# eddyxzc/lpopc

Hardware: AMD Instinct MI355X
Metric: eval_g+eval_jac_g calls/sec, 4-phase 4096-LGR-pt problem (higher is better)
Workload: dtype f64

## Files before the change

### lpopc_amd/csrc/rpm_ipm.hpp

```cpp
#pragma once
#include <string>
#include <vector>

#include "rpm_engine.hpp"

namespace rpm {

struct KktSubHost {
  int Nt, Nb, nb, b, CS;
  long long koff;
  int roff;
};

struct IpmPlan {
  int n = 0, m = 0, ns = 0, nv = 0;
  int Nt = 0, Nb = 0, nb = 0;
  int b = 0, CS = 0;
  std::vector<int> pos;
  std::vector<int> row_slack;
  std::vector<int> slack_row;
  std::vector<int> fixed;
  std::vector<int> jac_dst, hes_dst;
  std::vector<int> diag_dst;
  std::vector<int> slk_dst;
// ... 23 lines not shown
  }
};

int build_ipm_plan(Engine& e, IpmPlan& p, std::string* why, int nested = 0);
void ipm_plan_group_hessian(IpmPlan& p);
long long ipm_plan_offset(const IpmPlan& p, int ua, int uc);

#if defined(__HIP__) || defined(__HIPCC__)
#define RPM_IPM_HD __host__ __device__
#else
#define RPM_IPM_HD
#endif

constexpr int IPM_W = 16;
constexpr int IPM_LONG_COLUMN = 256;
constexpr int IPM_FILL_CHUNK = 4096;
constexpr int IPM_DENSE_SLOTS = 22, IPM_DENSE_TILE_WAVES = 7, IPM_DENSE_LDS_ROW = 18;
constexpr int IPM_DENSE_TILES = IPM_DENSE_SLOTS * IPM_DENSE_TILE_WAVES;
constexpr int IPM_DENSE_ROWS = 17, IPM_DENSE_EARLY = 4;
static_assert(IPM_DENSE_ROWS * (IPM_DENSE_ROWS + 1) / 2 <= IPM_DENSE_TILES, "resident tiles");
RPM_IPM_HD inline int ipm_dense_early(int block_rows) { return block_rows > IPM_DENSE_ROWS ? block_rows - IPM_DENSE_ROWS : 0; }
RPM_IPM_HD inline int ipm_dense_tile(int block_rows, int I, int Kb) {
  const int E = ipm_dense_early(block_rows), R = block_rows - E;
  if (Kb >= E) { const int kr = Kb - E; return kr * R - kr * (kr - 1) / 2 + I - Kb; }
  return R * (R + 1) / 2 + Kb * block_rows - Kb * (Kb - 1) / 2 + I - Kb;
}
RPM_IPM_HD inline int ipm_dense_tiles_of(int block_rows) { return block_rows * (block_rows + 1) / 2; }

inline size_t ipm_factor_lds_bytes(int b, int nb) {
  const size_t W = IPM_W;
// ... 21 lines not shown
struct IpmFillList {
  std::vector<int> dst, ki, hg, ptr;
  bool one_pass = false;
  int n_chunks() const { return one_pass ? int(ptr.size()) - 1 : 0; }
};
IpmFillList ipm_fill_list(const IpmPlan& p);

struct IpmFusedFill {
  bool built = false;
  int tiles = IPM_DENSE_TILES;
  std::vector<int> ptr, ki, hg, live;
  std::vector<unsigned long long> map;
};
IpmFusedFill ipm_fused_fill(const IpmSubList& s, const IpmFillList& fill);

}
```

### lpopc_amd/csrc/rpm_ipm_device.hpp

```cpp
#pragma once
#include <hip/hip_runtime.h>

#include "rpm_ipm.hpp"

namespace rpm {

constexpr int IPM_FMAX = 1024;
constexpr int IPM_TRACE = 8;
constexpr double IPM_INF = 1e19;
constexpr int IPM_LB_H = 6;
constexpr int IPM_LB_PART = 80 * 16;
constexpr int IPM_LB_SMALL = 8 + 2 * (2 * IPM_LB_H) * (2 * IPM_LB_H) + 2 * (2 * IPM_LB_H);

struct IpmOpts {
  double tol = 1e-8, mu_init = 0.1, kappa_eps = 10.0, kappa_mu = 0.2, theta_mu = 1.5, tau_min = 0.99;
  double bound_push = 1e-2, bound_frac = 1e-2, kappa_sigma = 1e10, s_max = 100.0;
  double ws_bound_push = 1e-3, ws_bound_frac = 1e-3, ws_slack_bound_push = 1e-3, ws_slack_bound_frac = 1e-3;
  double ws_mult_bound_push = 1e-3, ws_mult_init_max = 1e6;
  double gamma_theta = 1e-5, gamma_phi = 1e-8, eta_phi = 1e-8, delta = 1.0, s_theta = 1.1, s_phi = 2.3, gamma_alpha = 0.05;
  double delta_c = 1e-9, delta_w_first = 1e-4, delta_w_min = 1e-20, delta_w_max = 1e40, kw_inc_first = 100.0, kw_inc = 8.0,
         kw_dec = 1.0 / 3.0;
  int max_iter = 3000, max_ls = 40;
  double acceptable_tol = 1e-6;
  int acceptable_iter = 15;
// ... 20 lines not shown
  int status;
  int iter, nfilt, accepted, refactor, npos, nneg, nbad, ls, armijo, nzb, pad;
  int mode, resto_it, enter_resto, n_resto;
  int n_acc, skip_update;
  double th0, zeta;
  double mu_r, th_r, thr_max, thr_min, phi_r;
  int nrfilt, soc_on, soc_req, soc_p, use_soc, n_soc;
  double alpha_soc, az_soc, th_old_soc;
  double mu_max, refs[4];
  int fixed_mode, nrefs;
  int n_recalc, ic_hot;
  double th_trial, phi_trial;
  long long dbg[8];
};

struct IpmDev {
  int B, n, m, ns, nv, Nt, Nb, nb, b, CS, nnz_jac, nnz_h;
  long long sg, sv, kstride;
  const int *pos, *row_slack, *slack_row, *jac_dst, *hes_dst, *diag_dst, *slk_dst, *jt_ptr, *jt_ent, *jt_row;
  const int *hg_ptr, *hg_src, *hg_dst;
  int n_hg;
  const int *as_dst, *as_ki, *as_hg, *as_ptr;
  int as_nchunk;
  const int* long_cols;
  int n_long;
  const double *gl, *gu;
  double *v, *vl, *vu, *zL, *zU, *lam, *dv, *dlam, *dzL, *dzU, *glag, *c, *rhs, *K, *filt;
  double *xe, *xt, *grad, *g, *jac, *hess, *obj, *gt, *objt;
  double *vR, *dr2;
  double *vl0, *vu0;
// ... 7 lines not shown
  IpmInst* inst;
  int* cnt;
  IpmOpts o;
  const KktSub* subs;
  int n_sub, n_l1, n_l2;
  int* piv;
  const int *cg_ptr, *cg_src, *cg_dst;
  const int *rg_ptr, *rg_src, *rg_dst;
  const int *rs_dst, *rs_src;
  const int* gap_pos;
  int n_cg, n_rg, n_rs, n_gap;
  const int *cg2_ptr, *cg2_src, *cg2_dst, *rg2_ptr, *rg2_src, *rg2_dst, *rs2_dst, *rs2_src;
  int n_cg2, n_rg2, n_rs2;
  int n_cg_long, n_cg2_long;
  int max_sub_nt;
  int df_tiles;
  size_t l1_dense_lds;
  int last_dense_corner;
  size_t l2_dense_lds, last_dense_lds;
  int df_on;
  const int *df_ptr, *df_ki, *df_hg, *as_live;
  int as_nlive;
  const unsigned long long* df_map;
  int rhs_mult;
  int lb_on;
  double *lb_S, *lb_Y;
  double *lb_xprev;
  double *lb_gold;
  int scal_on;
  double *sc, *sf, *lam_h;
// ... 28 lines not shown
void ipm_launch_scale_lambda(const IpmDev& D, hipStream_t st);
void ipm_launch_scale_hessian(const IpmDev& D, hipStream_t st);
void ipm_launch_unscale_lambda(const IpmDev& D, double* out, hipStream_t st);
void lb_launch_reset(const IpmDev& D, hipStream_t st);
void lb_launch_update(const IpmDev& D, hipStream_t st);
void lb_launch_columns_and_solve(const IpmDev& D, hipStream_t st);
void lb_launch_small(const IpmDev& D, hipStream_t st);
void lb_launch_correct(const IpmDev& D, int check_status, hipStream_t st);
void ipm_launch_jt_lambda_into(const IpmDev& D, double* out, hipStream_t st);
size_t kkt_factor_lds_bytes(const IpmPlan& p);
hipError_t kkt_factor_prepare(int tiles_per_wave, size_t lds_bytes);
size_t kkt_factor_dense_lds_bytes(int block_rows);
int kkt_factor_dense_max_block_rows();
hipError_t kkt_factor_dense_prepare(size_t lds_bytes);
void kkt_launch_factor(const IpmDev& D, int tiles_per_wave, size_t lds_bytes, hipStream_t st);
void kkt_launch_solve(const IpmDev& D, int check_status, hipStream_t st, int forward_done = 0);
int kkt_level1_fused(const IpmDev& D);
void kkt_launch_vec(const IpmDev& D, unsigned n_rhs, const int* dst, const int* src, int n, int mode, int check_status, hipStream_t st);

}
```

### lpopc_amd/csrc/rpm_ipm_solver.hip

```cpp
#include <algorithm>
#include <cstdlib>
#include <cstring>
#include <memory>
#include <new>

#include "rpm_ipm_solver.hpp"

using namespace rpm;

namespace {
struct IpmAllocs {
  rpm_ipm* h;
  int rc = RPM_OK;
  template <class T>
  void room(T** dst, size_t count) { if (!rc) rc = ipm_alloc(h, dst, count); }
  template <class T>
  void table(const T** dst, const std::vector<T>& src) {
    T* p = nullptr;
    if (!rc) rc = ipm_alloc(h, &p, src.size(), src.data());
    *dst = p;
  }
};

bool env_is_zero(const char* name) {
// ... 36 lines not shown
    a.table(&D.as_live, fused.live); a.table(&D.df_map, fused.map);
    D.as_nlive = int(fused.live.size());
  }
  a.table(&D.subs, s.subs);
  D.n_sub = int(s.subs.size()); D.n_l1 = s.n_l1; D.n_l2 = s.n_l2; D.max_sub_nt = s.max_sub_nt;
  a.room(&D.piv, size_t(D.B) * s.subs.size() * 3);
  a.table(&D.cg_ptr, p.cg_ptr); a.table(&D.cg_src, p.cg_src); a.table(&D.cg_dst, p.cg_dst);
  a.table(&D.rg_ptr, p.rg_ptr); a.table(&D.rg_src, p.rg_src); a.table(&D.rg_dst, p.rg_dst);
  a.table(&D.rs_dst, p.rs_dst); a.table(&D.rs_src, p.rs_src); a.table(&D.gap_pos, p.gap_pos);
  D.n_cg = int(p.cg_dst.size()); D.n_rg = int(p.rg_dst.size()); D.n_rs = int(p.rs_dst.size()); D.n_gap = int(p.gap_pos.size());
  a.table(&D.cg2_ptr, p.cg2_ptr); a.table(&D.cg2_src, p.cg2_src); a.table(&D.cg2_dst, p.cg2_dst);
  a.table(&D.rg2_ptr, p.rg2_ptr); a.table(&D.rg2_src, p.rg2_src); a.table(&D.rg2_dst, p.rg2_dst);
  a.table(&D.rs2_dst, p.rs2_dst); a.table(&D.rs2_src, p.rs2_src);
  D.n_cg2 = int(p.cg2_dst.size()); D.n_rg2 = int(p.rg2_dst.size()); D.n_rs2 = int(p.rs2_dst.size());
  D.n_cg_long = p.n_cg_long; D.n_cg2_long = p.n_cg2_long;
  return a.rc;
}

int alloc_state(rpm_ipm* h) {
  Engine& e = h->eng->e;
  const IpmPlan& p = h->plan;
  IpmDev& D = h->D;
  const size_t B = size_t(D.B), Bm = B * size_t(std::max(p.m, 1));
  IpmAllocs a{h};
  a.room(&D.v, B * p.nv); a.room(&D.vl, B * p.nv); a.room(&D.vu, B * p.nv);
  a.room(&D.zL, B * p.nv); a.room(&D.zU, B * p.nv); a.room(&D.lam, B * p.m);
  a.room(&D.dv, B * p.nv); a.room(&D.dlam, B * p.m); a.room(&D.dzL, B * p.nv);
  a.room(&D.dzU, B * p.nv); a.room(&D.glag, B * p.nv); a.room(&D.c, B * p.m);
  a.room(&D.rhs, B * size_t(p.Nt_alloc)); a.room(&D.K, B * size_t(p.storage())); a.room(&D.filt, B * 2 * IPM_FMAX);
  a.room(&D.xe, B * p.n); a.room(&D.xt, B * p.n); a.room(&D.grad, B * p.n);
// ... 162 lines not shown
  }
  else if (k == "restoration_penalty") o.resto_rho = value;
  else if (k == "level1_dense") {
    if (value != 0.0 && !h->l1_dense_lds) { h->err = "level1_dense: no nested dissection, or an interval block of more than 21 block rows"; return RPM_E_UNSUPPORTED; }
    h->D.l1_dense_lds = value != 0.0 ? h->l1_dense_lds : 0;
  }
  else if (k == "upper_dense") {
    h->D.l2_dense_lds = value != 0.0 ? h->l2_dense_lds : 0;
    h->D.last_dense_lds = value != 0.0 ? h->last_dense_lds : 0;
    h->D.last_dense_corner = value == 2.0 ? 0 : 1;
  }
  else if (k == "fused_fill") {
    if (value != 0.0 && !h->D.df_map) { h->err = "fused_fill: level 1 does not run on kkt_factor_dense_kernel"; return RPM_E_UNSUPPORTED; }
    h->D.df_on = value != 0.0;
  }
  else if (k == "trace") {
    const int cap = int(value);
    if (cap < 0 || cap > 100000) { h->err = "trace: 0 ... 100000 records"; return RPM_E_INVALID; }
    h->D.trace = nullptr;
    h->D.trace_cap = 0;
    if (cap > 0) {
      int rc = ipm_alloc(h, &h->D.trace, size_t(h->D.B) * cap * IPM_TRACE);
      if (rc) return rc;
      h->D.trace_cap = cap;
    }
  }
  else { h->err = "unknown option " + k; return RPM_E_INVALID; }
  return RPM_OK;
}

// ... 325 lines not shown
```

### lpopc_amd/csrc/rpm_ipm_solver.hpp

```cpp
#pragma once
#include <algorithm>
#include <cstdio>
#include <string>
#include <vector>

#include "rpm_device_internal.hpp"
#include "rpm_ipm_device.hpp"

struct rpm_ipm {
  rpm_engine* eng = nullptr;
  rpm::IpmPlan plan;
  rpm::IpmDev D{};
  std::vector<void*> allocs;
  int* h_cnt = nullptr;
  size_t factor_lds = 0;
  size_t l1_dense_lds = 0;
  size_t l2_dense_lds = 0, last_dense_lds = 0;
  int factor_mt = rpm::IPM_MT;
  std::string err;
  std::vector<rpm::IpmInst> h_inst;
  int total_factorizations = 0, total_iterations = 0, total_trials = 0, total_soc = 0;
  hipEvent_t ev[4] = {nullptr, nullptr, nullptr, nullptr};
  double factor_ms = 0.0, solve_ms = 0.0;
  bool solve_pending = false;
  bool attached = false;
  bool lbfgs = false;
  int lb_iterations = 0;
  bool solved = false;
  bool debug_started = false;
  int debug_ls = 0;
  double* d_host_form = nullptr;
  ~rpm_ipm() {
    if (attached && eng && eng->e.ipm_attached > 0) eng->e.ipm_attached -= 1;
// ... 21 lines not shown
  IPM_TRY(h, hipMalloc(&p, (count ? count : 1) * sizeof(T)));
  h->allocs.push_back(p);
  *dst = static_cast<T*>(p);
  if (src && count) IPM_TRY(h, hipMemcpy(p, src, count * sizeof(T), hipMemcpyHostToDevice));
  return RPM_OK;
}

inline int launch_check(rpm_ipm* h, const char* what) {
  hipError_t s = hipGetLastError();
  if (s != hipSuccess) {
    h->err = std::string(what) + ": " + hipGetErrorString(s);
    return RPM_E_DEVICE;
  }
  return RPM_OK;
}
inline int factor_and_solve_launch(rpm_ipm* h, hipStream_t st, bool factor, bool solve, int check_status, int forward_done = 0) {
  if (factor) kkt_launch_factor(h->D, h->factor_mt, h->factor_lds, st);
  if (solve) kkt_launch_solve(h->D, check_status, st, forward_done);
  return launch_check(h, "kkt kernels");
}

int ipm_check_start_args(rpm_ipm* h, const char* who, const char* need, bool warm, const void* x, const void* lambda, const void* z_L,
                         const void* z_U);
int ipm_start(rpm_ipm* h, bool warm, const double* d_x, const double* d_lambda, const double* d_zL, const double* d_zU, hipStream_t st);
int host_form(rpm_ipm* h, double** d_x, double** d_l, double** d_zL, double** d_zU);

inline int ipm_abi_status(int device_status) {
  return device_status == 1 ? 0 : (device_status == 6 ? 1 : device_status);
}

struct IpmLoop {
  rpm_ipm* h;
  Engine& e;
// ... 35 lines not shown
      ipm_launch_inertia(D, st);
      h->total_factorizations += 1;
      if ((rc = fetch_counts())) return rc;
      float ms = 0.f;
      if (hipEventElapsedTime(&ms, h->ev[0], h->ev[1]) == hipSuccess) h->factor_ms += ms;
      if (h->h_cnt[1] == 0) break;
    }
    return RPM_OK;
  }
  int substitute() const {
    IPM_TRY(h, hipEventRecord(h->ev[2], st));
    if (h->lbfgs && h->lb_iterations > 0) {
      lb_launch_columns_and_solve(D, st);
      lb_launch_small(D, st);
    }
    if (int rc = factor_and_solve_launch(h, st, false, true, 1, 1)) return rc;
    if (h->lbfgs) lb_launch_correct(D, 1, st);
    IPM_TRY(h, hipEventRecord(h->ev[3], st));
    h->solve_pending = true;
    return RPM_OK;
  }
  int direction() const {
    IPM_TRY(h, hipMemsetAsync(D.cnt + 2, 0, 2 * sizeof(int), st));
    ipm_launch_direction(D, st);
    h->h_cnt[3] = 0;
    return RPM_OK;
  }
  int line_search_round(double* soc_rhs_copy = nullptr) const {
    int rc;
    if (h->h_cnt[3] > 0) {
      ipm_launch_soc_rhs(D, st);
      if (soc_rhs_copy)
        IPM_TRY(h, hipMemcpyAsync(soc_rhs_copy, D.rhs, size_t(D.B) * size_t(h->plan.Nt_alloc) * sizeof(double), hipMemcpyDeviceToHost, st));
      if ((rc = factor_and_solve_launch(h, st, false, true, 2))) return rc;
      if (h->lbfgs) lb_launch_correct(D, 2, st);
      ipm_launch_soc_direction(D, st);
      h->total_soc += 1;
    }
// ... 67 lines not shown
```

### lpopc_amd/csrc/rpm_ipm_tables.cpp

```cpp
#include <algorithm>
#include <unordered_map>

#include "rpm_ipm.hpp"

namespace rpm {

IpmSubList ipm_sub_list(const IpmPlan& p) {
  IpmSubList s;
  if (p.nd) {
    for (const KktSubHost& g : p.subs) s.subs.push_back(KktSub{KktGeom{g.Nt, g.Nb, g.nb, g.b, g.CS}, g.roff, g.koff});
    s.n_l2 = p.n_l2;
    s.n_l1 = int(s.subs.size()) - 1 - s.n_l2;
  } else {
    s.subs.push_back(KktSub{KktGeom{p.Nt, p.Nb, p.nb, p.b, p.CS}, 0, 0});
  }
  for (const KktSub& q : s.subs) s.max_sub_nt = std::max(s.max_sub_nt, q.g.Nt);
  return s;
}

std::vector<int> ipm_long_columns(const IpmPlan& p) {
  std::vector<int> cols;
  for (int i = 0; i < p.n; ++i)
    if (p.jt_ptr[size_t(i) + 1] - p.jt_ptr[size_t(i)] > IPM_LONG_COLUMN) cols.push_back(i);
  return cols;
// ... 77 lines not shown
        t.ki.push_back(fill.ki[q]);
        t.hg.push_back(fill.hg[q]);
      }
    }
    e2 = e3;
    if (size_t(number) + 1 > 2 * size_t(NTB) * IPM_W * IPM_DENSE_LDS_ROW) return none;
    for (long long c = (k0 + IPM_FILL_CHUNK - 1) / IPM_FILL_CHUNK; (c + 1) * IPM_FILL_CHUNK <= k1; ++c) skip[size_t(c)] = 1;
  }
  t.ptr[3 * size_t(s.n_l1)] = int(t.ki.size());
  for (int c = 0; c < fill.n_chunks(); ++c)
    if (!skip[size_t(c)]) t.live.push_back(c);
  t.built = true;
  return t;
}

}
```

### lpopc_amd/csrc/rpm_kkt_solve.hip

```cpp
#include <algorithm>
#include <cmath>
#include <cstring>
#include <new>

#include "rpm_device_internal.hpp"
#include "rpm_ipm_device.hpp"

namespace rpm {

__device__ inline void block_range(const KktGeom& G, int J0, int* J1, int* nrb, int* nr) {
  if (J0 < G.Nb) {
    *J1 = min(J0 + IPM_W, G.Nb);
    const int last = min(*J1 - 1 + G.b, G.Nb - 1);
    *nrb = max(last - *J1 + 1, 0);
    *nr = *nrb + G.nb;
  } else {
    *J1 = min(J0 + IPM_W, G.Nt);
    *nrb = 0;
    *nr = G.Nt - *J1;
  }
}
__device__ inline int panel_row(const KktGeom& G, int J0, int J1, int nrb, int q) {
  return J0 >= G.Nb ? J1 + q : (q < nrb ? J1 + q : G.Nb + (q - nrb));
}

template <bool RL, int PF = 1>
__global__ __launch_bounds__(256) void kkt_solve_kernel(const double* Kall, long long kstride, const KktSub* subs, int sub0, int n_here,
                                                        const IpmInst* inst, double* rhs_all, long long rhs_stride, int check_status,
                                                        int phase, int kmod) {
  constexpr int W = IPM_W;
#define SOLVE_BARRIER() do { if (RL) asm volatile("s_waitcnt lgkmcnt(0)\n\ts_barrier" ::: "memory"); else __syncthreads(); } while (0)
  const int bi = blockIdx.x / n_here, bk = bi % kmod, t = threadIdx.x, nt = blockDim.x;
  if (check_status && (inst[bk].status != 0 || (check_status == 2 && !inst[bk].soc_req))) return;
  const KktSub sub = subs[sub0 + int(blockIdx.x) % n_here];
  const KktGeom G = sub.g;
  const double* K = Kall + size_t(bk) * kstride + sub.koff;
  double* rg = rhs_all + size_t(bi) * rhs_stride + sub.roff;
  extern __shared__ double rsh[];
  double* r = RL ? rsh : rg;
  __shared__ double Dg[W * (W + 1)], ys[W], zs[W], red[4][W];
  const int di = t / W, dj = t % W;
  const int nbb = (G.Nb + W - 1) / W, ncb = (G.nb + W - 1) / W, nblk = nbb + ncb;
  if (RL) {
    for (int i = t; i < G.Nt; i += nt) rsh[i] = rg[i];
    SOLVE_BARRIER();
  }
  struct Blk { int J0, J1, nrb, nr, w; };
  auto blk_of = [&](int blk) {
    Blk B;
    B.J0 = blk < nbb ? blk * W : G.Nb + (blk - nbb) * W;
    block_range(G, B.J0, &B.J1, &B.nrb, &B.nr);
    B.w = B.J1 - B.J0;
    return B;
  };
  auto fetch = [&](int blk, double& dg, double (&l)[W]) {
    if (blk < 0 || blk >= nblk) return;
    const Blk B = blk_of(blk);
    dg = (di < B.w && dj <= di) ? K[G.at(B.J0 + di, B.J0 + dj)] : 0.0;
    const int row = t < B.nr ? panel_row(G, B.J0, B.J1, B.nrb, t) : -1;
    const bool brd = row >= G.Nb;
    const int kstep = brd ? G.CS : G.CS - 1;
    const double* kp = K + (size_t(B.J0) * G.CS + (brd ? G.b + 1 + row - G.Nb : max(row - B.J0, 0)));
#pragma unroll
    for (int c = 0; c < W; ++c)
      l[c] = (row >= 0 && c < B.w && (brd || row - (B.J0 + c) <= G.b)) ? kp[c * kstep] : 0.0;
  };
  double dg0, l0[W], dg1, l1[W];
  const int fwd_end = phase == 1 ? nbb : (phase == 2 ? 0 : nblk), bwd_begin = phase == 2 ? nbb : (phase == 1 ? 0 : nblk);
  auto forward_step = [&](int blk, double& dg, double (&l)[W]) {
    const Blk B = blk_of(blk);
    if (di < W && dj <= di) Dg[di * (W + 1) + dj] = dg;
    if (t < W) zs[t] = t < B.w ? r[B.J0 + t] : 0.0;
    SOLVE_BARRIER();
    if (t < W) {
      double y = zs[t];
#pragma unroll
      for (int k = 0; k < W; ++k)
        if (k < t && t < B.w) y = __builtin_fma(Dg[t * (W + 1) + k], zs[k], y);
      ys[t] = y;
      if (t < B.w) r[B.J0 + t] = y;
    }
    SOLVE_BARRIER();
    for (int q = t; q < B.nr; q += nt) {
      const int row = panel_row(G, B.J0, B.J1, B.nrb, q);
      double acc = 0.0;
#pragma unroll
      for (int c = 0; c < W; ++c) {
        const double lv = q == t ? l[c] : ((c < B.w && (row >= G.Nb || row - (B.J0 + c) <= G.b)) ? K[G.at(row, B.J0 + c)] : 0.0);
        acc = __builtin_fma(lv, ys[c], acc);
      }
      r[row] -= acc;
    }
    fetch(blk + PF, dg, l);
    SOLVE_BARRIER();
  };
  if (fwd_end > 0) { fetch(0, dg0, l0); if (PF == 2) fetch(1 < fwd_end ? 1 : -1, dg1, l1); }
  for (int blk = 0; blk < fwd_end; blk += PF) {
    forward_step(blk, dg0, l0);
    if (PF == 2 && blk + 1 < fwd_end) forward_step(blk + 1, dg1, l1);
  }
  auto backward_step = [&](int blk, double& dg, double (&l)[W]) {
    const Blk B = blk_of(blk);
    if (di < W && dj <= di) Dg[di * (W + 1) + dj] = dg;
    double p[W];
#pragma unroll
    for (int c = 0; c < W; ++c) p[c] = 0.0;
    for (int q = t; q < B.nr; q += nt) {
      const int row = panel_row(G, B.J0, B.J1, B.nrb, q);
      const double xr = r[row];
#pragma unroll
      for (int c = 0; c < W; ++c) {
        const double lv = q == t ? l[c] : ((c < B.w && (row >= G.Nb || row - (B.J0 + c) <= G.b)) ? K[G.at(row, B.J0 + c)] : 0.0);
        p[c] = __builtin_fma(lv, xr, p[c]);
      }
    }
    fetch(blk - PF, dg, l);
    {
      const int ln = t & 63;
      double q8[8], q4[4], q2[2], u;
      const bool h32 = ln & 32, h16 = ln & 16, h8 = ln & 8, h4 = ln & 4;
#pragma unroll
      for (int i = 0; i < 8; ++i) q8[i] = (h32 ? p[i + 8] : p[i]) + __shfl_xor(h32 ? p[i] : p[i + 8], 32);
#pragma unroll
      for (int i = 0; i < 4; ++i) q4[i] = (h16 ? q8[i + 4] : q8[i]) + __shfl_xor(h16 ? q8[i] : q8[i + 4], 16);
#pragma unroll
      for (int i = 0; i < 2; ++i) q2[i] = (h8 ? q4[i + 2] : q4[i]) + __shfl_xor(h8 ? q4[i] : q4[i + 2], 8);
      u = (h4 ? q2[1] : q2[0]) + __shfl_xor(h4 ? q2[0] : q2[1], 4);
      u += __shfl_xor(u, 2);
      u += __shfl_xor(u, 1);
      if ((ln & 3) == 0) red[t >> 6][ln >> 2] = u;
    }
    SOLVE_BARRIER();
    if (t < W) zs[t] = t < B.w ? r[B.J0 + t] / Dg[t * (W + 1) + t] - (red[0][t] + red[1][t] + red[2][t] + red[3][t]) : 0.0;
    SOLVE_BARRIER();
    if (t < B.w) {
      double x = zs[t];
#pragma unroll
      for (int k = 0; k < W; ++k)
        if (k > t && k < B.w) x = __builtin_fma(Dg[k * (W + 1) + t], zs[k], x);
      r[B.J0 + t] = x;
    }
    SOLVE_BARRIER();
  };
  if (bwd_begin > 0) { fetch(bwd_begin - 1, dg0, l0); if (PF == 2) fetch(bwd_begin - 2, dg1, l1); }
  for (int blk = bwd_begin - 1; blk >= 0; blk -= PF) {
    backward_step(blk, dg0, l0);
    if (PF == 2 && blk - 1 >= 0) backward_step(blk - 1, dg1, l1);
  }
  if (RL)
    for (int i = t; i < G.Nt; i += nt) rg[i] = rsh[i];
#undef SOLVE_BARRIER
}

__global__ __launch_bounds__(256) void ipm_inertia_kernel(IpmDev D) {
  const int bi = (blockIdx.x * blockDim.x + threadIdx.x) >> 6, lane = threadIdx.x & 63;
  if (bi >= D.B) return;
  IpmInst& S = D.inst[bi];
  if (S.status != 0 || !S.refactor) return;
  const IpmOpts& o = D.o;
// ... 36 lines not shown
}
__global__ void kkt_vec_kernel(double* vall, long long vstride, const int* __restrict__ dst, const int* __restrict__ src, int n, int mode,
                               const IpmInst* inst, int check_status, int kmod) {
  const int bi = blockIdx.y, bk = bi % kmod;
  if (check_status && (inst[bk].status != 0 || (check_status == 2 && !inst[bk].soc_req) || (check_status == 3 && !inst[bk].refactor))) return;
  double* v = vall + size_t(bi) * vstride;
  for (int i = blockIdx.x * blockDim.x + threadIdx.x; i < n; i += gridDim.x * blockDim.x) v[dst[i]] = mode ? v[src[i]] : 0.0;
}
void kkt_launch_vec(const IpmDev& D, unsigned n_rhs, const int* dst, const int* src, int n, int mode, int check_status, hipStream_t st) {
  if (!n) return;
  const unsigned blocks = unsigned(std::max(1, std::min(256, (n + 255) / 256)));
  hipLaunchKernelGGL(kkt_vec_kernel, dim3(blocks, n_rhs), dim3(256), 0, st, D.rhs, (long long)D.Nt, dst, src, n, mode, D.inst,
                     check_status, D.B);
}

static void launch_solve_subs(const IpmDev& D, int sub0, int n_here, int phase, int check_status, hipStream_t st) {
  const dim3 grid(unsigned(D.B) * unsigned(D.rhs_mult > 1 ? D.rhs_mult : 1) * unsigned(n_here));
  if (size_t(D.max_sub_nt) * sizeof(double) <= 48 * 1024 && grid.x <= 512)
    hipLaunchKernelGGL((kkt_solve_kernel<true, 2>), grid, dim3(256), size_t(D.max_sub_nt) * sizeof(double), st, D.K, D.kstride, D.subs, sub0, n_here,
                       D.inst, D.rhs, (long long)D.Nt, check_status, phase, D.B);
  else if (size_t(D.max_sub_nt) * sizeof(double) <= 48 * 1024)
    hipLaunchKernelGGL(kkt_solve_kernel<true>, grid, dim3(256), size_t(D.max_sub_nt) * sizeof(double), st, D.K, D.kstride, D.subs, sub0, n_here,
                       D.inst, D.rhs, (long long)D.Nt, check_status, phase, D.B);
  else
    hipLaunchKernelGGL(kkt_solve_kernel<false>, grid, dim3(256), 0, st, D.K, D.kstride, D.subs, sub0, n_here, D.inst, D.rhs, (long long)D.Nt,
                       check_status, phase, D.B);
}
void kkt_launch_solve(const IpmDev& D, int check_status, hipStream_t st, int forward_done) {
  const unsigned VB = unsigned(D.B) * unsigned(D.rhs_mult > 1 ? D.rhs_mult : 1);
  if (D.n_l1 == 0) {
    launch_solve_subs(D, 0, 1, 0, check_status, st);
    return;
  }
  auto vec = [&](const int* dst, const int* src, int n, int mode) { kkt_launch_vec(D, VB, dst, src, n, mode, check_status, st); };
  auto gather = [&](const int* ptr, const int* src, const int* dst, int n) {
    if (!n) return;
    const unsigned blocks = unsigned(std::max(1, std::min(4096, (n + 3) / 4)));
    hipLaunchKernelGGL(kkt_gather_seq_kernel, dim3(blocks, VB), dim3(256), 0, st, D.rhs, (long long)D.Nt, ptr, src, dst, n, D.inst, check_status, D.B);
  };
  if (!(forward_done && kkt_level1_fused(D))) {
    vec(D.gap_pos, nullptr, D.n_gap, 0);
    launch_solve_subs(D, 0, D.n_l1, 1, check_status, st);
  }
  gather(D.rg_ptr, D.rg_src, D.rg_dst, D.n_rg);
  if (D.n_l2) {
    launch_solve_subs(D, D.n_l1, D.n_l2, 1, check_status, st);
    gather(D.rg2_ptr, D.rg2_src, D.rg2_dst, D.n_rg2);
  }
  launch_solve_subs(D, D.n_l1 + D.n_l2, 1, 0, check_status, st);
  if (D.n_l2) {
    vec(D.rs2_dst, D.rs2_src, D.n_rs2, 1);
    launch_solve_subs(D, D.n_l1, D.n_l2, 2, check_status, st);
  }
  vec(D.rs_dst, D.rs_src, D.n_rs, 1);
  launch_solve_subs(D, 0, D.n_l1, 2, check_status, st);
}
void ipm_launch_inertia(const IpmDev& D, hipStream_t st) {
  hipLaunchKernelGGL(ipm_inertia_kernel, dim3(unsigned((D.B + 3) / 4)), dim3(256), 0, st, D);
}

}
```

Before: 653,900.

## Fuse inter-level KKT gather/copy glue and step staging into solve kernels

After: 651,600. No clear change (-0.3%).

```diff
diff --git a/lpopc_amd/csrc/rpm_ipm.hpp b/lpopc_amd/csrc/rpm_ipm.hpp
--- a/lpopc_amd/csrc/rpm_ipm.hpp
+++ b/lpopc_amd/csrc/rpm_ipm.hpp
@@ -61,6 +61,7 @@
 
 constexpr int IPM_W = 16;
 constexpr int IPM_LONG_COLUMN = 256;
+constexpr int IPM_GLUE_LONG = 16;
 constexpr int IPM_FILL_CHUNK = 4096;
 constexpr int IPM_DENSE_SLOTS = 22, IPM_DENSE_TILE_WAVES = 7, IPM_DENSE_LDS_ROW = 18;
 constexpr int IPM_DENSE_TILES = IPM_DENSE_SLOTS * IPM_DENSE_TILE_WAVES;
@@ -112,4 +113,11 @@
 };
 IpmFusedFill ipm_fused_fill(const IpmSubList& s, const IpmFillList& fill);
 
+struct IpmGlueTables {
+  bool built = false;
+  std::vector<int> g_sub, g_ptr, g_src, g_dst, c_sub, c_dst, c_src;
+  std::vector<int> l_ptr[2], l_src[2], l_dst[2];
+};
+IpmGlueTables ipm_glue_tables(const IpmPlan& p, const IpmSubList& s);
+
 }
diff --git a/lpopc_amd/csrc/rpm_ipm_device.hpp b/lpopc_amd/csrc/rpm_ipm_device.hpp
--- a/lpopc_amd/csrc/rpm_ipm_device.hpp
+++ b/lpopc_amd/csrc/rpm_ipm_device.hpp
@@ -58,6 +58,11 @@
   long long dbg[8];
 };
 
+struct KktGlue {
+  const int *g_sub, *g_ptr, *g_src, *g_dst, *c_sub, *c_dst, *c_src;
+  int on;
+};
+
 struct IpmDev {
   int B, n, m, ns, nv, Nt, Nb, nb, b, CS, nnz_jac, nnz_h;
   long long sg, sv, kstride;
@@ -95,6 +100,11 @@
   int n_cg2, n_rg2, n_rs2;
   int n_cg_long, n_cg2_long;
   int max_sub_nt;
+  KktGlue glue;
+  const int *gl_ptr[2], *gl_src[2], *gl_dst[2];
+  int n_gl[2];
+  int fused_steps;
+  int fused_sub;
   int df_tiles;
   size_t l1_dense_lds;
   int last_dense_corner;
@@ -153,7 +163,7 @@
 int kkt_factor_dense_max_block_rows();
 hipError_t kkt_factor_dense_prepare(size_t lds_bytes);
 void kkt_launch_factor(const IpmDev& D, int tiles_per_wave, size_t lds_bytes, hipStream_t st);
-void kkt_launch_solve(const IpmDev& D, int check_status, hipStream_t st, int forward_done = 0);
+void kkt_launch_solve(const IpmDev& D, int check_status, hipStream_t st, int forward_done = 0, int* zero_cnt = nullptr, int n_zero_cnt = 0);
 int kkt_level1_fused(const IpmDev& D);
 void kkt_launch_vec(const IpmDev& D, unsigned n_rhs, const int* dst, const int* src, int n, int mode, int check_status, hipStream_t st);
 
diff --git a/lpopc_amd/csrc/rpm_ipm_solver.hip b/lpopc_amd/csrc/rpm_ipm_solver.hip
--- a/lpopc_amd/csrc/rpm_ipm_solver.hip
+++ b/lpopc_amd/csrc/rpm_ipm_solver.hip
@@ -74,6 +74,19 @@
   a.table(&D.rs2_dst, p.rs2_dst); a.table(&D.rs2_src, p.rs2_src);
   D.n_cg2 = int(p.cg2_dst.size()); D.n_rg2 = int(p.rg2_dst.size()); D.n_rs2 = int(p.rs2_dst.size());
   D.n_cg_long = p.n_cg_long; D.n_cg2_long = p.n_cg2_long;
+  const IpmGlueTables glue = ipm_glue_tables(p, s);
+  h->glue_built = glue.built;
+  if (glue.built) {
+    a.table(&D.glue.g_sub, glue.g_sub); a.table(&D.glue.g_ptr, glue.g_ptr); a.table(&D.glue.g_src, glue.g_src); a.table(&D.glue.g_dst, glue.g_dst);
+    a.table(&D.glue.c_sub, glue.c_sub); a.table(&D.glue.c_dst, glue.c_dst); a.table(&D.glue.c_src, glue.c_src);
+    for (int st = 0; st < 2; ++st) {
+      a.table(&D.gl_ptr[st], glue.l_ptr[st]); a.table(&D.gl_src[st], glue.l_src[st]); a.table(&D.gl_dst[st], glue.l_dst[st]);
+      D.n_gl[st] = int(glue.l_dst[st].size());
+    }
+  }
+  D.fused_sub = 1;
+  D.fused_steps = 1;
+  D.glue.on = glue.built ? 1 : 0;
   return a.rc;
 }
 
@@ -266,6 +279,11 @@
     if (value != 0.0 && !h->D.df_map) { h->err = "fused_fill: level 1 does not run on kkt_factor_dense_kernel"; return RPM_E_UNSUPPORTED; }
     h->D.df_on = value != 0.0;
   }
+  else if (k == "fused_substitution") {
+    h->D.fused_sub = value == 1.0 || value == 3.0;
+    h->D.fused_steps = value == 1.0 || value == 2.0;
+    h->D.glue.on = h->D.fused_sub && h->glue_built;
+  }
   else if (k == "trace") {
     const int cap = int(value);
     if (cap < 0 || cap > 100000) { h->err = "trace: 0 ... 100000 records"; return RPM_E_INVALID; }
diff --git a/lpopc_amd/csrc/rpm_ipm_solver.hpp b/lpopc_amd/csrc/rpm_ipm_solver.hpp
--- a/lpopc_amd/csrc/rpm_ipm_solver.hpp
+++ b/lpopc_amd/csrc/rpm_ipm_solver.hpp
@@ -17,6 +17,7 @@
   size_t l1_dense_lds = 0;
   size_t l2_dense_lds = 0, last_dense_lds = 0;
   int factor_mt = rpm::IPM_MT;
+  bool glue_built = false;
   std::string err;
   std::vector<rpm::IpmInst> h_inst;
   int total_factorizations = 0, total_iterations = 0, total_trials = 0, total_soc = 0;
@@ -68,9 +69,10 @@
   }
   return RPM_OK;
 }
-inline int factor_and_solve_launch(rpm_ipm* h, hipStream_t st, bool factor, bool solve, int check_status, int forward_done = 0) {
+inline int factor_and_solve_launch(rpm_ipm* h, hipStream_t st, bool factor, bool solve, int check_status, int forward_done = 0,
+                                   int* zero_cnt = nullptr, int n_zero_cnt = 0) {
   if (factor) kkt_launch_factor(h->D, h->factor_mt, h->factor_lds, st);
-  if (solve) kkt_launch_solve(h->D, check_status, st, forward_done);
+  if (solve) kkt_launch_solve(h->D, check_status, st, forward_done, zero_cnt, n_zero_cnt);
   return launch_check(h, "kkt kernels");
 }
 
@@ -136,14 +138,14 @@
       lb_launch_columns_and_solve(D, st);
       lb_launch_small(D, st);
     }
-    if (int rc = factor_and_solve_launch(h, st, false, true, 1, 1)) return rc;
+    if (int rc = factor_and_solve_launch(h, st, false, true, 1, 1, D.fused_sub ? D.cnt + 2 : nullptr, 2)) return rc;
     if (h->lbfgs) lb_launch_correct(D, 1, st);
     IPM_TRY(h, hipEventRecord(h->ev[3], st));
     h->solve_pending = true;
     return RPM_OK;
   }
   int direction() const {
-    IPM_TRY(h, hipMemsetAsync(D.cnt + 2, 0, 2 * sizeof(int), st));
+    if (!D.fused_sub) IPM_TRY(h, hipMemsetAsync(D.cnt + 2, 0, 2 * sizeof(int), st));
     ipm_launch_direction(D, st);
     h->h_cnt[3] = 0;
     return RPM_OK;
diff --git a/lpopc_amd/csrc/rpm_ipm_tables.cpp b/lpopc_amd/csrc/rpm_ipm_tables.cpp
--- a/lpopc_amd/csrc/rpm_ipm_tables.cpp
+++ b/lpopc_amd/csrc/rpm_ipm_tables.cpp
@@ -115,4 +115,105 @@
   return t;
 }
 
-}
+IpmGlueTables ipm_glue_tables(const IpmPlan& p, const IpmSubList& s) {
+  IpmGlueTables none, t;
+  const int n_sub = int(s.subs.size());
+  if (s.n_l1 <= 0 || n_sub != s.n_l1 + s.n_l2 + 1) return none;
+  auto level_of = [&](int si) { return si < s.n_l1 ? 1 : (si < s.n_l1 + s.n_l2 ? 2 : 3); };
+  auto sub_of = [&](int row) {
+    int lo = 0, hi = n_sub;
+    while (hi - lo > 1) {
+      const int mid = (lo + hi) / 2;
+      if (s.subs[size_t(mid)].roff <= row) lo = mid; else hi = mid;
+    }
+    const KktSub& q = s.subs[size_t(lo)];
+    return row >= q.roff && row < q.roff + q.g.Nt ? lo : -1;
+  };
+  for (int si = 1; si < n_sub; ++si)
+    if (s.subs[size_t(si)].roff < s.subs[size_t(si) - 1].roff + s.subs[size_t(si) - 1].g.Nt) return none;
+  auto in_work_space = [&](int row, int si) { return si >= 0 && level_of(si) < 3 && row >= s.subs[size_t(si)].roff + s.subs[size_t(si)].g.Nb; };
+
+  {
+    size_t rows = 0;
+    for (int si = 0; si < s.n_l1 + s.n_l2; ++si) rows += size_t(s.subs[size_t(si)].g.nb);
+    if (p.gap_pos.size() != rows) return none;
+    std::vector<int> g = p.gap_pos;
+    std::sort(g.begin(), g.end());
+    for (size_t i = 0; i < g.size(); ++i)
+      if ((i > 0 && g[i] == g[i - 1]) || !in_work_space(g[i], sub_of(g[i]))) return none;
+  }
+
+  struct Dest { int sub, row; bool in_stage[2]; std::vector<int> src[2]; };
+  std::vector<Dest> dests;
+  std::unordered_map<int, size_t> dest_of_row;
+  auto add_stage = [&](const std::vector<int>& ptr, const std::vector<int>& src, const std::vector<int>& dst, int src_level) {
+    if (ptr.size() != dst.size() + 1 && !(dst.empty() && ptr.empty())) return false;
+    std::unordered_map<int, int> seen;
+    for (size_t i = 0; i < dst.size(); ++i) {
+      const int si = sub_of(dst[i]);
+      if (si < 0 || level_of(si) <= src_level || in_work_space(dst[i], si) || !seen.emplace(dst[i], 1).second) return false;
+      if (ptr[i] < 0 || ptr[i] > ptr[i + 1] || size_t(ptr[i + 1]) > src.size()) return false;
+      auto it = dest_of_row.find(dst[i]);
+      if (it == dest_of_row.end()) {
+        it = dest_of_row.emplace(dst[i], dests.size()).first;
+        dests.push_back(Dest{si, dst[i], {false, false}, {{}, {}}});
+      }
+      dests[it->second].in_stage[src_level - 1] = true;
+      for (int j = ptr[i]; j < ptr[i + 1]; ++j) {
+        const int ss = sub_of(src[size_t(j)]);
+        if (ss < 0 || level_of(ss) != src_level || !in_work_space(src[size_t(j)], ss)) return false;
+        dests[it->second].src[src_level - 1].push_back(src[size_t(j)]);
+      }
+    }
+    return true;
+  };
+  if (!add_stage(p.rg_ptr, p.rg_src, p.rg_dst, 1)) return none;
+  if (!add_stage(p.rg2_ptr, p.rg2_src, p.rg2_dst, 2)) return none;
+  std::stable_sort(dests.begin(), dests.end(), [](const Dest& a, const Dest& b) { return a.sub < b.sub; });
+  t.g_sub.assign(size_t(n_sub) + 1, 0);
+  t.g_ptr.push_back(0);
+  for (int st = 0; st < 2; ++st) t.l_ptr[st].push_back(0);
+  for (const Dest& d : dests) {
+    if (d.src[0].size() > size_t(IPM_GLUE_LONG) || d.src[1].size() > size_t(IPM_GLUE_LONG)) {
+      for (int st = 0; st < 2; ++st) {
+        if (!d.in_stage[st]) continue;
+        t.l_dst[st].push_back(d.row);
+        t.l_src[st].insert(t.l_src[st].end(), d.src[st].begin(), d.src[st].end());
+        t.l_ptr[st].push_back(int(t.l_src[st].size()));
+      }
+      continue;
+    }
+    t.g_sub[size_t(d.sub) + 1] += 1;
+    t.g_dst.push_back(d.row);
+    for (int st = 0; st < 2; ++st) t.g_src.insert(t.g_src.end(), d.src[st].begin(), d.src[st].end());
+    t.g_ptr.push_back(int(t.g_src.size()));
+  }
+  for (int si = 0; si < n_sub; ++si) t.g_sub[size_t(si) + 1] += t.g_sub[size_t(si)];
+
+  struct Copy { int sub, dst, src; };
+  std::vector<Copy> copies;
+  std::unordered_map<int, int> copied;
+  auto add_copies = [&](const std::vector<int>& dst, const std::vector<int>& src, int dst_level) {
+    if (dst.size() != src.size()) return false;
+    for (size_t i = 0; i < dst.size(); ++i) {
+      const int sd = sub_of(dst[i]), ss = sub_of(src[i]);
+      if (sd < 0 || level_of(sd) != dst_level || !in_work_space(dst[i], sd) || !copied.emplace(dst[i], 1).second) return false;
+      if (ss < 0 || level_of(ss) <= dst_level || in_work_space(src[i], ss)) return false;
+      copies.push_back(Copy{sd, dst[i], src[i]});
+    }
+    return true;
+  };
+  if (!add_copies(p.rs_dst, p.rs_src, 1) || !add_copies(p.rs2_dst, p.rs2_src, 2)) return none;
+  std::stable_sort(copies.begin(), copies.end(), [](const Copy& a, const Copy& b) { return a.sub < b.sub; });
+  t.c_sub.assign(size_t(n_sub) + 1, 0);
+  for (const Copy& c : copies) {
+    t.c_sub[size_t(c.sub) + 1] += 1;
+    t.c_dst.push_back(c.dst);
+    t.c_src.push_back(c.src);
+  }
+  for (int si = 0; si < n_sub; ++si) t.c_sub[size_t(si) + 1] += t.c_sub[size_t(si)];
+  t.built = true;
+  return t;
+}
+
+}
diff --git a/lpopc_amd/csrc/rpm_kkt_solve.hip b/lpopc_amd/csrc/rpm_kkt_solve.hip
--- a/lpopc_amd/csrc/rpm_kkt_solve.hip
+++ b/lpopc_amd/csrc/rpm_kkt_solve.hip
@@ -24,26 +24,83 @@
   return J0 >= G.Nb ? J1 + q : (q < nrb ? J1 + q : G.Nb + (q - nrb));
 }
 
-template <bool RL, int PF = 1>
+__device__ inline double lane_value(double v, int k) {
+  return __hiloint2double(__builtin_amdgcn_readlane(__double2hiint(v), k), __builtin_amdgcn_readlane(__double2loint(v), k));
+}
+
+template <bool RL, int PF = 1, bool FS = false>
 __global__ __launch_bounds__(256) void kkt_solve_kernel(const double* Kall, long long kstride, const KktSub* subs, int sub0, int n_here,
                                                         const IpmInst* inst, double* rhs_all, long long rhs_stride, int check_status,
-                                                        int phase, int kmod) {
+                                                        int phase, int kmod, KktGlue glue, int* zero_cnt, int n_zero_cnt) {
   constexpr int W = IPM_W;
 #define SOLVE_BARRIER() do { if (RL) asm volatile("s_waitcnt lgkmcnt(0)\n\ts_barrier" ::: "memory"); else __syncthreads(); } while (0)
   const int bi = blockIdx.x / n_here, bk = bi % kmod, t = threadIdx.x, nt = blockDim.x;
-  if (check_status && (inst[bk].status != 0 || (check_status == 2 && !inst[bk].soc_req))) return;
-  const KktSub sub = subs[sub0 + int(blockIdx.x) % n_here];
+  if (zero_cnt && blockIdx.x == 0 && t < n_zero_cnt) zero_cnt[t] = 0;
+  const int si = sub0 + int(blockIdx.x) % n_here;
+  const KktSub sub = subs[si];
+  const bool gathers = glue.on && phase != 2, copies = glue.on && phase == 2;
+  const int* list_of = gathers ? glue.g_sub : glue.c_sub;
+  const int list0 = glue.on ? list_of[si] : 0, list1 = glue.on ? list_of[si + 1] : 0;
+  const int inst_status = check_status ? inst[bk].status : 0, inst_soc = check_status == 2 ? inst[bk].soc_req : 1;
+  if (inst_status != 0 || !inst_soc) return;
   const KktGeom G = sub.g;
   const double* K = Kall + size_t(bk) * kstride + sub.koff;
   double* rg = rhs_all + size_t(bi) * rhs_stride + sub.roff;
   extern __shared__ double rsh[];
   double* r = RL ? rsh : rg;
-  __shared__ double Dg[W * (W + 1)], ys[W], zs[W], red[4][W];
+  __shared__ double Dg2[(FS ? 2 : 1) * W * (W + 1)], ys[W], zs[W], red[4][W];
   const int di = t / W, dj = t % W;
   const int nbb = (G.Nb + W - 1) / W, ncb = (G.nb + W - 1) / W, nblk = nbb + ncb;
+  constexpr int GB = 8;
+  const double* v = rhs_all + size_t(bi) * rhs_stride;
+  auto gather_fetch = [&](int j, int j1, double (&s)[GB]) {
+    int idx[GB];
+#pragma unroll
+    for (int u = 0; u < GB; ++u) idx[u] = j + u < j1 ? glue.g_src[j + u] : -1;
+#pragma unroll
+    for (int u = 0; u < GB; ++u) s[u] = idx[u] >= 0 ? v[idx[u]] : 0.0;
+  };
+  auto gather_add = [&](int j, int j1, const double (&s)[GB], double acc) {
+#pragma unroll
+    for (int u = 0; u < GB; ++u)
+      if (j + u < j1) acc += s[u];
+    return acc;
+  };
+  const bool zero_border = glue.on && phase == 1;
+  const int e0 = list0 + t, e1 = list1;
+  int gj0 = 0, gj1 = 0, gd = 0;
+  double gs[GB], cv = 0.0;
+  if (gathers && e0 < e1) {
+    gj0 = glue.g_ptr[e0]; gj1 = glue.g_ptr[e0 + 1]; gd = glue.g_dst[e0] - sub.roff;
+    gather_fetch(gj0, gj1, gs);
+  }
+  if (copies && e0 < e1) { gd = glue.c_dst[e0] - sub.roff; cv = v[glue.c_src[e0]]; }
   if (RL) {
-    for (int i = t; i < G.Nt; i += nt) rsh[i] = rg[i];
-    SOLVE_BARRIER();
+    for (int i = t; i < G.Nt; i += nt) rsh[i] = (zero_border && i >= G.Nb) ? 0.0 : rg[i];
+    SOLVE_BARRIER();
+  } else if (zero_border) {
+    for (int i = G.Nb + t; i < G.Nt; i += nt) rg[i] = 0.0;
+    __syncthreads();
+  }
+  if (glue.on) {
+    for (int e = e0; e < e1; e += nt) {
+      if (e != e0) {
+        if (gathers) { gj0 = glue.g_ptr[e]; gj1 = glue.g_ptr[e + 1]; gd = glue.g_dst[e] - sub.roff; gather_fetch(gj0, gj1, gs); }
+        else { gd = glue.c_dst[e] - sub.roff; cv = v[glue.c_src[e]]; }
+      }
+      if (gathers) {
+        double acc = gather_add(gj0, gj1, gs, r[gd]);
+        for (int j = gj0 + GB; j < gj1; j += GB) {
+          double s[GB];
+          gather_fetch(j, gj1, s);
+          acc = gather_add(j, gj1, s, acc);
+        }
+        r[gd] = acc;
+      } else {
+        r[gd] = cv;
+      }
+    }
+    __syncthreads();
   }
   struct Blk { int J0, J1, nrb, nr, w; };
   auto blk_of = [&](int blk) {
@@ -53,10 +110,18 @@
     B.w = B.J1 - B.J0;
     return B;
   };
-  auto fetch = [&](int blk, double& dg, double (&l)[W]) {
+  auto fetch_dg = [&](int blk, double& dg) {
     if (blk < 0 || blk >= nblk) return;
     const Blk B = blk_of(blk);
     dg = (di < B.w && dj <= di) ? K[G.at(B.J0 + di, B.J0 + dj)] : 0.0;
+  };
+  auto stage_dg = [&](int blk, double dg) {
+    if (dj <= di) Dg2[(FS ? (blk & 1) : 0) * W * (W + 1) + di * (W + 1) + dj] = dg;
+  };
+  auto fetch = [&](int blk, int ahead, double& dg, double (&l)[W]) {
+    fetch_dg(blk + ahead, dg);
+    if (blk < 0 || blk >= nblk) return;
+    const Blk B = blk_of(blk);
     const int row = t < B.nr ? panel_row(G, B.J0, B.J1, B.nrb, t) : -1;
     const bool brd = row >= G.Nb;
     const int kstep = brd ? G.CS : G.CS - 1;
@@ -65,18 +130,24 @@
     for (int c = 0; c < W; ++c)
       l[c] = (row >= 0 && c < B.w && (brd || row - (B.J0 + c) <= G.b)) ? kp[c * kstep] : 0.0;
   };
-  double dg0, l0[W], dg1, l1[W];
+  double dg0 = 0.0, l0[W], dg1 = 0.0, l1[W];
   const int fwd_end = phase == 1 ? nbb : (phase == 2 ? 0 : nblk), bwd_begin = phase == 2 ? nbb : (phase == 1 ? 0 : nblk);
   auto forward_step = [&](int blk, double& dg, double (&l)[W]) {
     const Blk B = blk_of(blk);
-    if (di < W && dj <= di) Dg[di * (W + 1) + dj] = dg;
-    if (t < W) zs[t] = t < B.w ? r[B.J0 + t] : 0.0;
-    SOLVE_BARRIER();
+    const double* Dg = Dg2 + (FS ? (blk & 1) : 0) * W * (W + 1);
+    if (!FS) {
+      stage_dg(blk, dg);
+      if (t < W) zs[t] = t < B.w ? r[B.J0 + t] : 0.0;
+      SOLVE_BARRIER();
+    }
     if (t < W) {
-      double y = zs[t];
-#pragma unroll
-      for (int k = 0; k < W; ++k)
-        if (k < t && t < B.w) y = __builtin_fma(Dg[t * (W + 1) + k], zs[k], y);
+      const double z = FS ? (t < B.w ? r[B.J0 + t] : 0.0) : zs[t];
+      double y = z;
+#pragma unroll
+      for (int k = 0; k < W; ++k) {
+        const double zk = FS ? lane_value(z, k) : zs[k];
+        if (k < t && t < B.w) y = __builtin_fma(Dg[t * (W + 1) + k], zk, y);
+      }
       ys[t] = y;
       if (t < B.w) r[B.J0 + t] = y;
     }
@@ -91,17 +162,27 @@
       }
       r[row] -= acc;
     }
-    fetch(blk + PF, dg, l);
-    SOLVE_BARRIER();
-  };
-  if (fwd_end > 0) { fetch(0, dg0, l0); if (PF == 2) fetch(1 < fwd_end ? 1 : -1, dg1, l1); }
+    if (FS) stage_dg(blk + 1, dg);
+    fetch(blk + PF, FS ? 1 : 0, dg, l);
+    SOLVE_BARRIER();
+  };
+  auto prime_dg = [&](int blk) {
+    double d0 = 0.0;
+    fetch_dg(blk, d0);
+    stage_dg(blk, d0);
+    __syncthreads();
+  };
+  if (FS && fwd_end > 0) prime_dg(0);
+  if (fwd_end > 0) { fetch(0, FS ? 1 : 0, dg0, l0); if (PF == 2) fetch(1 < fwd_end ? 1 : -1 - nblk, FS ? 1 : 0, dg1, l1); }
   for (int blk = 0; blk < fwd_end; blk += PF) {
     forward_step(blk, dg0, l0);
     if (PF == 2 && blk + 1 < fwd_end) forward_step(blk + 1, dg1, l1);
   }
   auto backward_step = [&](int blk, double& dg, double (&l)[W]) {
     const Blk B = blk_of(blk);
-    if (di < W && dj <= di) Dg[di * (W + 1) + dj] = dg;
+    const double* Dg = Dg2 + (FS ? (blk & 1) : 0) * W * (W + 1);
+    if (FS) { if (blk > 0) stage_dg(blk - 1, dg); }
+    else stage_dg(blk, dg);
     double p[W];
 #pragma unroll
     for (int c = 0; c < W; ++c) p[c] = 0.0;
@@ -114,7 +195,7 @@
         p[c] = __builtin_fma(lv, xr, p[c]);
       }
     }
-    fetch(blk - PF, dg, l);
+    fetch(blk - PF, FS ? -1 : 0, dg, l);
     {
       const int ln = t & 63;
       double q8[8], q4[4], q2[2], u;
@@ -131,18 +212,25 @@
       if ((ln & 3) == 0) red[t >> 6][ln >> 2] = u;
     }
     SOLVE_BARRIER();
-    if (t < W) zs[t] = t < B.w ? r[B.J0 + t] / Dg[t * (W + 1) + t] - (red[0][t] + red[1][t] + red[2][t] + red[3][t]) : 0.0;
-    SOLVE_BARRIER();
+    double z = 0.0;
+    if (t < W) {
+      z = t < B.w ? r[B.J0 + t] / Dg[t * (W + 1) + t] - (red[0][t] + red[1][t] + red[2][t] + red[3][t]) : 0.0;
+      if (!FS) zs[t] = z;
+    }
+    if (!FS) SOLVE_BARRIER();
     if (t < B.w) {
-      double x = zs[t];
-#pragma unroll
-      for (int k = 0; k < W; ++k)
-        if (k > t && k < B.w) x = __builtin_fma(Dg[k * (W + 1) + t], zs[k], x);
+      double x = FS ? z : zs[t];
+#pragma unroll
+      for (int k = 0; k < W; ++k) {
+        const double zk = FS ? lane_value(z, k) : zs[k];
+        if (k > t && k < B.w) x = __builtin_fma(Dg[k * (W + 1) + t], zk, x);
+      }
       r[B.J0 + t] = x;
     }
     SOLVE_BARRIER();
   };
-  if (bwd_begin > 0) { fetch(bwd_begin - 1, dg0, l0); if (PF == 2) fetch(bwd_begin - 2, dg1, l1); }
+  if (FS && bwd_begin > 0) prime_dg(bwd_begin - 1);
+  if (bwd_begin > 0) { fetch(bwd_begin - 1, FS ? -1 : 0, dg0, l0); if (PF == 2) fetch(bwd_begin - 2, FS ? -1 : 0, dg1, l1); }
   for (int blk = bwd_begin - 1; blk >= 0; blk -= PF) {
     backward_step(blk, dg0, l0);
     if (PF == 2 && blk - 1 >= 0) backward_step(blk - 1, dg1, l1);
@@ -209,22 +297,27 @@
                      check_status, D.B);
 }
 
-static void launch_solve_subs(const IpmDev& D, int sub0, int n_here, int phase, int check_status, hipStream_t st) {
+static void launch_solve_subs(const IpmDev& D, int sub0, int n_here, int phase, int check_status, hipStream_t st, int* zero_cnt = nullptr,
+                              int n_zero_cnt = 0) {
   const dim3 grid(unsigned(D.B) * unsigned(D.rhs_mult > 1 ? D.rhs_mult : 1) * unsigned(n_here));
-  if (size_t(D.max_sub_nt) * sizeof(double) <= 48 * 1024 && grid.x <= 512)
-    hipLaunchKernelGGL((kkt_solve_kernel<true, 2>), grid, dim3(256), size_t(D.max_sub_nt) * sizeof(double), st, D.K, D.kstride, D.subs, sub0, n_here,
-                       D.inst, D.rhs, (long long)D.Nt, check_status, phase, D.B);
-  else if (size_t(D.max_sub_nt) * sizeof(double) <= 48 * 1024)
-    hipLaunchKernelGGL(kkt_solve_kernel<true>, grid, dim3(256), size_t(D.max_sub_nt) * sizeof(double), st, D.K, D.kstride, D.subs, sub0, n_here,
-                       D.inst, D.rhs, (long long)D.Nt, check_status, phase, D.B);
-  else
-    hipLaunchKernelGGL(kkt_solve_kernel<false>, grid, dim3(256), 0, st, D.K, D.kstride, D.subs, sub0, n_here, D.inst, D.rhs, (long long)D.Nt,
-                       check_status, phase, D.B);
-}
-void kkt_launch_solve(const IpmDev& D, int check_status, hipStream_t st, int forward_done) {
+  const size_t rhs_bytes = size_t(D.max_sub_nt) * sizeof(double);
+  const bool in_lds = rhs_bytes <= 48 * 1024;
+  auto launch = [&](auto kernel) {
+    hipLaunchKernelGGL(kernel, grid, dim3(256), in_lds ? rhs_bytes : 0, st, D.K, D.kstride, D.subs, sub0, n_here, D.inst, D.rhs, (long long)D.Nt,
+                       check_status, phase, D.B, D.glue, zero_cnt, n_zero_cnt);
+  };
+  if (in_lds && grid.x <= 512) {
+    if (D.fused_steps) launch(kkt_solve_kernel<true, 2, true>); else launch(kkt_solve_kernel<true, 2, false>);
+  } else if (in_lds) {
+    if (D.fused_steps) launch(kkt_solve_kernel<true, 1, true>); else launch(kkt_solve_kernel<true, 1, false>);
+  } else {
+    if (D.fused_steps) launch(kkt_solve_kernel<false, 1, true>); else launch(kkt_solve_kernel<false, 1, false>);
+  }
+}
+void kkt_launch_solve(const IpmDev& D, int check_status, hipStream_t st, int forward_done, int* zero_cnt, int n_zero_cnt) {
   const unsigned VB = unsigned(D.B) * unsigned(D.rhs_mult > 1 ? D.rhs_mult : 1);
   if (D.n_l1 == 0) {
-    launch_solve_subs(D, 0, 1, 0, check_status, st);
+    launch_solve_subs(D, 0, 1, 0, check_status, st, zero_cnt, n_zero_cnt);
     return;
   }
   auto vec = [&](const int* dst, const int* src, int n, int mode) { kkt_launch_vec(D, VB, dst, src, n, mode, check_status, st); };
@@ -233,6 +326,16 @@
     const unsigned blocks = unsigned(std::max(1, std::min(4096, (n + 3) / 4)));
     hipLaunchKernelGGL(kkt_gather_seq_kernel, dim3(blocks, VB), dim3(256), 0, st, D.rhs, (long long)D.Nt, ptr, src, dst, n, D.inst, check_status, D.B);
   };
+  if (D.glue.on) {
+    if (!(forward_done && kkt_level1_fused(D))) launch_solve_subs(D, 0, D.n_l1, 1, check_status, st);
+    gather(D.gl_ptr[0], D.gl_src[0], D.gl_dst[0], D.n_gl[0]);
+    if (D.n_l2) launch_solve_subs(D, D.n_l1, D.n_l2, 1, check_status, st);
+    gather(D.gl_ptr[1], D.gl_src[1], D.gl_dst[1], D.n_gl[1]);
+    launch_solve_subs(D, D.n_l1 + D.n_l2, 1, 0, check_status, st);
+    if (D.n_l2) launch_solve_subs(D, D.n_l1, D.n_l2, 2, check_status, st);
+    launch_solve_subs(D, 0, D.n_l1, 2, check_status, st, zero_cnt, n_zero_cnt);
+    return;
+  }
   if (!(forward_done && kkt_level1_fused(D))) {
     vec(D.gap_pos, nullptr, D.n_gap, 0);
     launch_solve_subs(D, 0, D.n_l1, 1, check_status, st);
@@ -248,7 +351,7 @@
     launch_solve_subs(D, D.n_l1, D.n_l2, 2, check_status, st);
   }
   vec(D.rs_dst, D.rs_src, D.n_rs, 1);
-  launch_solve_subs(D, 0, D.n_l1, 2, check_status, st);
+  launch_solve_subs(D, 0, D.n_l1, 2, check_status, st, zero_cnt, n_zero_cnt);
 }
 void ipm_launch_inertia(const IpmDev& D, hipStream_t st) {
   hipLaunchKernelGGL(ipm_inertia_kernel, dim3(unsigned((D.B + 3) / 4)), dim3(256), 0, st, D);
```
